# jie0530/act-plus-plus

Hardware: AMD Instinct MI355X
Metric: policy steps/sec (4x480x640 cams, chunk=100, bs=8) (higher is better)
Workload: dtype f32 (f16x3 split products: 3 fp16 MFMAs per fp32 product, fp32 accumulate); 1 GPU; ACT eval policy query: 4 cams 480x640 u8, chunk 100, hidden 512, ff 3200, 4 enc + 7 dec layers (layer 0 live), per-GPU batch 8, + temporal ensemble; per_gpu_batch=8, global_batch=8, parallelism=replicas x1

## Files before the change

act-plus-plus_amd/csrc/attn.hip:

```cpp
#include "common.h"
#include "dropout.h"
#include "split16.h"
#include <cstdio>
#include <cstdlib>

namespace {

constexpr bool ATTN_NOPF = true;
constexpr int KT = 64;
typedef _Float16 h16x8 __attribute__((ext_vector_type(8)));

__device__ __forceinline__ void attn_block_coords(int& bx, int& by, int& bz) {
    const int gx = gridDim.x, gy = gridDim.y;
    const int total = gx * gy * (int)gridDim.z;
    const int lin = ((int)blockIdx.z * gy + (int)blockIdx.y) * gx + (int)blockIdx.x;
    const int xcd = lin & 7, q = total >> 3, r = total & 7;
    const int base = (xcd < r) ? xcd * (q + 1) : r * (q + 1) + (xcd - r) * q;
    const int flat = base + (lin >> 3);
    bx = flat % gx;
    const int rest = flat / gx;
    by = rest % gy;
    bz = rest / gy;
}

template <int HD>
__global__ __launch_bounds__(256) void attn_f32_kernel(AttnArgs p, int nsplit, int chunk) {
    constexpr int HH = HD / 2;
    constexpr int DT = (HD + 31) / 32;
    constexpr int VD = DT * 32;
    constexpr int KS = HD + 4;
    __shared__ __attribute__((aligned(16))) float s_k[KT * KS];
    __shared__ __attribute__((aligned(16))) float s_v[KT * VD];

    const int t = threadIdx.x, lane = t & 63, wave = t >> 6;
    const int li = lane & 31, lh = lane >> 5;
    int bx, h, b;
    attn_block_coords(bx, h, b);
    const int split = bx % nsplit;
    const int q = (bx / nsplit) * 128 + wave * 32 + li;
    const int k_begin = split * chunk;
    const int k_end = (k_begin + chunk < p.Nk) ? k_begin + chunk : p.Nk;
    const bool qok = q < p.Nq;

    const float qscale = p.scale * 1.4426950408889634f;
    const float* Qp = p.Q + (int64_t)b * p.q_bs + (int64_t)(qok ? q : 0) * p.q_rs + h * HD + lh * HH;
    float qreg[HH];
#pragma unroll
    for (int s = 0; s < HH; s += 4) {
        f32x4 v = *reinterpret_cast<const f32x4*>(Qp + s);
#pragma unroll
        for (int j = 0; j < 4; ++j) qreg[s + j] = qok ? v[j] * qscale : 0.f;
    }
    const float* Kb = p.K + (int64_t)b * p.k_bs + h * HD;
    const float* Vb = p.V + (int64_t)b * p.v_bs + h * HD;
    const uint8_t* kpm = p.kpm ? p.kpm + (int64_t)b * p.kpm_bs : nullptr;

    f32x16 O[DT];
#pragma unroll
    for (int d = 0; d < DT; ++d)
#pragma unroll
        for (int e = 0; e < 16; ++e) O[d][e] = 0.f;
    float m_run = -INFINITY, l_run = 0.f;

    if (HD < VD) {
        for (int e = t; e < KT * VD; e += 256) s_v[e] = 0.f;
        __syncthreads();
    }

    __shared__ uint8_t s_dead[KT];
    constexpr int C4 = HD / 4;
    constexpr int NLD = (KT * C4 + 255) / 256;
    f32x4 pk[NLD], pv[NLD];
    auto fetch = [&](int kt0) {
#pragma unroll
        for (int i = 0; i < NLD; ++i) {
            const int e = t + 256 * i;
            const int kr = e / C4, c = e - kr * C4;
            const int key = kt0 + kr;
            const bool ok = e < KT * C4 && key < k_end;
            const int64_t koff = ok ? (int64_t)key * p.k_rs + c * 4 : 0;
            const int64_t voff = ok ? (int64_t)key * p.v_rs + c * 4 : 0;
            const f32x4 kv = *reinterpret_cast<const f32x4*>(Kb + koff);
            const f32x4 vv = *reinterpret_cast<const f32x4*>(Vb + voff);
            const f32x4 z = {0.f, 0.f, 0.f, 0.f};
            pk[i] = ok ? kv : z;
            pv[i] = ok ? vv : z;
        }
    };
    fetch(k_begin);
    for (int kt0 = k_begin; kt0 < k_end; kt0 += KT) {
#pragma unroll
        for (int i = 0; i < NLD; ++i) {
            const int e = t + 256 * i;
            if (e < KT * C4) {
                const int kr = e / C4, c = e - kr * C4;
                *reinterpret_cast<f32x4*>(&s_k[kr * KS + c * 4]) = pk[i];
                *reinterpret_cast<f32x4*>(&s_v[kr * VD + c * 4]) = pv[i];
            }
        }
        const bool ragged = kt0 + KT > k_end || kpm != nullptr;
        if (ragged && t < KT) {
            const int key = kt0 + t;
            s_dead[t] = (key >= k_end) || (kpm && kpm[key] != 0);
        }
        __syncthreads();
        if (kt0 + KT < k_end) fetch(kt0 + KT);
#pragma unroll
        for (int sub = 0; sub < KT / 32; ++sub) {
            const int kb = kt0 + sub * 32;
            if (kb < k_end) {
                f32x16 S;
#pragma unroll
                for (int e = 0; e < 16; ++e) S[e] = 0.f;
                const float* krow = &s_k[(sub * 32 + li) * KS + lh * HH];
#pragma unroll
                for (int s = 0; s < HH; s += 4) {
                    const f32x4 kv = *reinterpret_cast<const f32x4*>(krow + s);
#pragma unroll
                    for (int j = 0; j < 4; ++j)
                        S = __builtin_amdgcn_mfma_f32_32x32x2f32(kv[j], qreg[s + j], S, 0, 0, 0);
                }
                if (ragged) {
#pragma unroll
                    for (int e = 0; e < 16; ++e)
                        if (s_dead[sub * 32 + (e & 3) + 8 * (e >> 2) + 4 * lh]) S[e] = -INFINITY;
                }
                if (p.causal) {
#pragma unroll
                    for (int e = 0; e < 16; ++e)
                        if (kb + (e & 3) + 8 * (e >> 2) + 4 * lh > q) S[e] = -INFINITY;
                }
                float mt = S[0];
#pragma unroll
                for (int e = 1; e < 16; ++e) mt = fmaxf(mt, S[e]);
                mt = fmaxf(mt, __shfl_xor(mt, 32, 64));
                const float m_new = fmaxf(m_run, mt);
                const float m_safe = (m_new == -INFINITY) ? 0.f : m_new;
                const float alpha = __builtin_amdgcn_exp2f(m_run - m_safe);
                float rs = 0.f;
#pragma unroll
                for (int e = 0; e < 16; ++e) {
                    S[e] = __builtin_amdgcn_exp2f(S[e] - m_safe);
                    rs += S[e];
                }
                rs += __shfl_xor(rs, 32, 64);
                l_run = l_run * alpha + rs;
                m_run = m_new;
                if (p.drop_p > 0.f) {
                    const float ds = 1.f / (1.f - p.drop_p);
                    const uint64_t rowbase = (((uint64_t)b * p.H + h) * p.Nq + (qok ? q : 0)) * (uint64_t)p.Nk;
#pragma unroll
                    for (int e = 0; e < 16; ++e) {
                        const int key = kb + (e & 3) + 8 * (e >> 2) + 4 * lh;
                        S[e] = actmi_keep(p.drop_seed, rowbase + key, p.drop_p) ? S[e] * ds : 0.f;
                    }
                }
#pragma unroll
                for (int d = 0; d < DT; ++d)
#pragma unroll
                    for (int e = 0; e < 16; ++e) O[d][e] *= alpha;
#pragma unroll
                for (int e = 0; e < 16; ++e) {
                    const int kl = sub * 32 + (e & 3) + 8 * (e >> 2) + 4 * lh;
#pragma unroll
                    for (int d = 0; d < DT; ++d) {
                        const float vv = s_v[kl * VD + d * 32 + li];
                        O[d] = __builtin_amdgcn_mfma_f32_32x32x2f32(vv, S[e], O[d], 0, 0, 0);
                    }
                }
            }
        }
        __syncthreads();
    }
    if (qok) {
        if (nsplit == 1) {
            const float inv = 1.f / l_run;
            float* Op = p.O + (int64_t)b * p.o_bs + (int64_t)q * p.o_rs + h * HD;
#pragma unroll
            for (int d = 0; d < DT; ++d)
#pragma unroll
                for (int g = 0; g < 4; ++g) {
                    const int d0 = d * 32 + 8 * g + 4 * lh;
                    if (d0 < HD) {
                        f32x4 o = {O[d][4 * g] * inv, O[d][4 * g + 1] * inv, O[d][4 * g + 2] * inv, O[d][4 * g + 3] * inv};
                        *reinterpret_cast<f32x4*>(Op + d0) = o;
                    }
                }
            if (p.lse && lh == 0) p.lse[((int64_t)b * p.H + h) * p.Nq + q] = m_run * 0.6931471805599453f + logf(l_run);
        } else {
            const int64_t row = (((int64_t)split * p.B + b) * p.H + h) * p.Nq + q;
            float* Op = p.ws + row * HD;
            float* ml = p.ws + (int64_t)nsplit * p.B * p.H * p.Nq * HD + row * 2;
#pragma unroll
            for (int d = 0; d < DT; ++d)
#pragma unroll
                for (int g = 0; g < 4; ++g) {
                    const int d0 = d * 32 + 8 * g + 4 * lh;
                    if (d0 < HD) {
                        f32x4 o = {O[d][4 * g], O[d][4 * g + 1], O[d][4 * g + 2], O[d][4 * g + 3]};
                        *reinterpret_cast<f32x4*>(Op + d0) = o;
                    }
                }
            if (lh == 0) { ml[0] = m_run; ml[1] = l_run; }
        }
    }
}

template <int HD>
__global__ __launch_bounds__(256, 3) void attn_f16x3_kernel(AttnArgs p, int nsplit, int chunk) {
    constexpr int NS = HD / 16;
    constexpr int DT = (HD + 31) / 32;
    constexpr int VD = DT * 32;
    constexpr int KROW = 4 * HD + 16;
    constexpr int VROW = 4 * KT + 16;
    __shared__ __attribute__((aligned(16))) unsigned char s_k[KT * KROW];
    __shared__ __attribute__((aligned(16))) unsigned char s_vt[VD * VROW];
    __shared__ uint8_t s_dead[KT];

    const int t = threadIdx.x, lane = t & 63, wave = t >> 6;
    const int li = lane & 31, lh = lane >> 5;
    int bx, h, b;
    attn_block_coords(bx, h, b);
    const int split = bx % nsplit;
    const int q = (bx / nsplit) * 128 + wave * 32 + li;
    const int k_begin = split * chunk;
    const int k_end = (k_begin + chunk < p.Nk) ? k_begin + chunk : p.Nk;
    const bool qok = q < p.Nq;

    const float qscale = p.scale * 1.4426950408889634f;
    const float* Qp = p.Q + (int64_t)b * p.q_bs + (int64_t)(qok ? q : 0) * p.q_rs + h * HD + lh * 8;
    h16x8 qh[NS], ql[NS];
#pragma unroll
    for (int s = 0; s < NS; ++s) {
        f32x4 v0 = *reinterpret_cast<const f32x4*>(Qp + s * 16);
        f32x4 v1 = *reinterpret_cast<const f32x4*>(Qp + s * 16 + 4);
        const float sc = qok ? qscale : 0.f;
        v0 *= sc; v1 *= sc;
        uint2 h0, l0, h1, l1;
        split16(v0, h0, l0);
        split16(v1, h1, l1);
        qh[s] = __builtin_bit_cast(h16x8, uint4{h0.x, h0.y, h1.x, h1.y});
        ql[s] = __builtin_bit_cast(h16x8, uint4{l0.x, l0.y, l1.x, l1.y});
    }
    const float* Kb = p.K + (int64_t)b * p.k_bs + h * HD;
    const float* Vb = p.V + (int64_t)b * p.v_bs + h * HD;
    const uint8_t* kpm = p.kpm ? p.kpm + (int64_t)b * p.kpm_bs : nullptr;

    f32x16 O[DT];
#pragma unroll
    for (int d = 0; d < DT; ++d)
#pragma unroll
        for (int e = 0; e < 16; ++e) O[d][e] = 0.f;
    float m_run = -INFINITY, l_run = 0.f;

    if (HD < VD) {
        for (int e = t; e < VD * VROW / 4; e += 256) reinterpret_cast<uint32_t*>(s_vt)[e] = 0u;
        __syncthreads();
    }

    constexpr int C4 = HD / 4;
    constexpr int NLK = (KT * C4 + 255) / 256;
    constexpr int NLV = (KT / 2 * C4 + 255) / 256;
    f32x4 pk[NLK], pv[NLV][2];
    auto vc = [&](int e) { return ((e >> 5) % (C4 / 4)) * 4 + (e & 3); };
    auto vkp = [&](int e) { return ((e >> 5) / (C4 / 4)) * 8 + ((e >> 2) & 7); };
    auto fetch = [&](int kt0) {
        const f32x4 z = {0.f, 0.f, 0.f, 0.f};
#pragma unroll
        for (int i = 0; i < NLK; ++i) {
            const int e = t + 256 * i;
            const int kr = e / C4, c = e - kr * C4;
            const int key = kt0 + kr;
            const bool ok = e < KT * C4 && key < k_end;
            const f32x4 kv = *reinterpret_cast<const f32x4*>(Kb + (ok ? (int64_t)key * p.k_rs + c * 4 : 0));
            pk[i] = ok ? kv : z;
        }
#pragma unroll
        for (int i = 0; i < NLV; ++i) {
            const int e = t + 256 * i;
            const int kp = vkp(e), c = vc(e);
#pragma unroll
            for (int u = 0; u < 2; ++u) {
                const int key = kt0 + 2 * kp + u;
                const bool ok = e < KT / 2 * C4 && key < k_end;
                const f32x4 vv = *reinterpret_cast<const f32x4*>(Vb + (ok ? (int64_t)key * p.v_rs + c * 4 : 0));
                pv[i][u] = ok ? vv : z;
            }
        }
    };
    if (!ATTN_NOPF) fetch(k_begin);
    for (int kt0 = k_begin; kt0 < k_end; kt0 += KT) {
        if (ATTN_NOPF) fetch(kt0);
#pragma unroll
        for (int i = 0; i < NLK; ++i) {
            const int e = t + 256 * i;
            if (e < KT * C4) {
                const int kr = e / C4, c = e - kr * C4;
                uint2 hi, lo;
                split16(pk[i], hi, lo);
                *reinterpret_cast<uint2*>(s_k + kr * KROW + c * 8) = hi;
                *reinterpret_cast<uint2*>(s_k + kr * KROW + 2 * HD + c * 8) = lo;
            }
        }
#pragma unroll
        for (int i = 0; i < NLV; ++i) {
            const int e = t + 256 * i;
            if (e < KT / 2 * C4) {
                const int kp = vkp(e), c = vc(e);
                uint2 ha, la, hb, lb;
                split16(pv[i][0], ha, la);
                split16(pv[i][1], hb, lb);
                const int kl = 2 * kp, r = kl & 15;
                const int pos = (kl & ~15) | (r & 3) | ((r & 8) >> 1) | ((r & 4) << 1);
                unsigned char* dst = s_vt + (c * 4) * VROW + pos * 2;
                *reinterpret_cast<uint32_t*>(dst + 0 * VROW) = (ha.x & 0xffffu) | (hb.x << 16);
                *reinterpret_cast<uint32_t*>(dst + 1 * VROW) = (ha.x >> 16) | (hb.x & 0xffff0000u);
                *reinterpret_cast<uint32_t*>(dst + 2 * VROW) = (ha.y & 0xffffu) | (hb.y << 16);
                *reinterpret_cast<uint32_t*>(dst + 3 * VROW) = (ha.y >> 16) | (hb.y & 0xffff0000u);
                *reinterpret_cast<uint32_t*>(dst + 0 * VROW + 2 * KT) = (la.x & 0xffffu) | (lb.x << 16);
                *reinterpret_cast<uint32_t*>(dst + 1 * VROW + 2 * KT) = (la.x >> 16) | (lb.x & 0xffff0000u);
                *reinterpret_cast<uint32_t*>(dst + 2 * VROW + 2 * KT) = (la.y & 0xffffu) | (lb.y << 16);
                *reinterpret_cast<uint32_t*>(dst + 3 * VROW + 2 * KT) = (la.y >> 16) | (lb.y & 0xffff0000u);
            }
        }
        const bool ragged = kt0 + KT > k_end || kpm != nullptr;
        if (ragged && t < KT) {
            const int key = kt0 + t;
            s_dead[t] = (key >= k_end) || (kpm && kpm[key] != 0);
        }
        __syncthreads();
        if (!ATTN_NOPF && kt0 + KT < k_end) fetch(kt0 + KT);
#pragma unroll
        for (int sub = 0; sub < KT / 32; ++sub) {
            const int kb = kt0 + sub * 32;
            if (kb < k_end) {
                f32x16 S;
#pragma unroll
                for (int e = 0; e < 16; ++e) S[e] = 0.f;
                const unsigned char* krow = s_k + (sub * 32 + li) * KROW + lh * 16;
#pragma unroll
                for (int s = 0; s < NS; ++s) {
                    const h16x8 kh = __builtin_bit_cast(h16x8, *reinterpret_cast<const f32x4*>(krow + s * 32));
                    const h16x8 kl = __builtin_bit_cast(h16x8, *reinterpret_cast<const f32x4*>(krow + 2 * HD + s * 32));
                    S = __builtin_amdgcn_mfma_f32_32x32x16_f16(kl, qh[s], S, 0, 0, 0);
                    S = __builtin_amdgcn_mfma_f32_32x32x16_f16(kh, ql[s], S, 0, 0, 0);
                    S = __builtin_amdgcn_mfma_f32_32x32x16_f16(kh, qh[s], S, 0, 0, 0);
                }
                if (ragged) {
#pragma unroll
                    for (int e = 0; e < 16; ++e)
                        if (s_dead[sub * 32 + (e & 3) + 8 * (e >> 2) + 4 * lh]) S[e] = -INFINITY;
                }
                if (p.causal) {
#pragma unroll
                    for (int e = 0; e < 16; ++e)
                        if (kb + (e & 3) + 8 * (e >> 2) + 4 * lh > q) S[e] = -INFINITY;
                }
                float mt = S[0];
#pragma unroll
                for (int e = 1; e < 16; ++e) mt = fmaxf(mt, S[e]);
                mt = fmaxf(mt, __shfl_xor(mt, 32, 64));
                const float m_new = fmaxf(m_run, mt);
                const float m_safe = (m_new == -INFINITY) ? 0.f : m_new;
                const float alpha = __builtin_amdgcn_exp2f(m_run - m_safe);
                float rs = 0.f;
#pragma unroll
                for (int e = 0; e < 16; ++e) {
                    S[e] = __builtin_amdgcn_exp2f(S[e] - m_safe);
                    rs += S[e];
                }
                rs += __shfl_xor(rs, 32, 64);
                l_run = l_run * alpha + rs;
                m_run = m_new;
                if (p.drop_p > 0.f) {
                    const float ds = 1.f / (1.f - p.drop_p);
                    const uint64_t rowbase = (((uint64_t)b * p.H + h) * p.Nq + (qok ? q : 0)) * (uint64_t)p.Nk;
#pragma unroll
                    for (int e = 0; e < 16; ++e) {
                        const int key = kb + (e & 3) + 8 * (e >> 2) + 4 * lh;
                        S[e] = actmi_keep(p.drop_seed, rowbase + key, p.drop_p) ? S[e] * ds : 0.f;
                    }
                }
                h16x8 ph[2], pl[2];
#pragma unroll
                for (int g2 = 0; g2 < 2; ++g2) {
                    const f32x4 a0 = {S[8 * g2], S[8 * g2 + 1], S[8 * g2 + 2], S[8 * g2 + 3]};
                    const f32x4 a1 = {S[8 * g2 + 4], S[8 * g2 + 5], S[8 * g2 + 6], S[8 * g2 + 7]};
                    uint2 h0, l0, h1, l1;
                    split16(a0, h0, l0);
                    split16(a1, h1, l1);
                    ph[g2] = __builtin_bit_cast(h16x8, uint4{h0.x, h0.y, h1.x, h1.y});
                    pl[g2] = __builtin_bit_cast(h16x8, uint4{l0.x, l0.y, l1.x, l1.y});
                }
#pragma unroll
                for (int d = 0; d < DT; ++d) {
#pragma unroll
                    for (int e = 0; e < 16; ++e) O[d][e] *= alpha;
                    const unsigned char* vrow = s_vt + (d * 32 + li) * VROW + sub * 64 + lh * 16;
#pragma unroll
                    for (int g2 = 0; g2 < 2; ++g2) {
                        const h16x8 vh = __builtin_bit_cast(h16x8, *reinterpret_cast<const f32x4*>(vrow + g2 * 32));
                        const h16x8 vl = __builtin_bit_cast(h16x8, *reinterpret_cast<const f32x4*>(vrow + 2 * KT + g2 * 32));
                        O[d] = __builtin_amdgcn_mfma_f32_32x32x16_f16(vl, ph[g2], O[d], 0, 0, 0);
                        O[d] = __builtin_amdgcn_mfma_f32_32x32x16_f16(vh, pl[g2], O[d], 0, 0, 0);
                        O[d] = __builtin_amdgcn_mfma_f32_32x32x16_f16(vh, ph[g2], O[d], 0, 0, 0);
                    }
                }
            }
        }
        __syncthreads();
    }
    if (qok) {
        if (nsplit == 1) {
            const float inv = 1.f / l_run;
            float* Op = p.O + (int64_t)b * p.o_bs + (int64_t)q * p.o_rs + h * HD;
#pragma unroll
            for (int d = 0; d < DT; ++d)
#pragma unroll
                for (int g = 0; g < 4; ++g) {
                    const int d0 = d * 32 + 8 * g + 4 * lh;
                    if (d0 < HD) {
                        f32x4 o = {O[d][4 * g] * inv, O[d][4 * g + 1] * inv, O[d][4 * g + 2] * inv, O[d][4 * g + 3] * inv};
                        *reinterpret_cast<f32x4*>(Op + d0) = o;
                    }
                }
            if (p.lse && lh == 0) p.lse[((int64_t)b * p.H + h) * p.Nq + q] = m_run * 0.6931471805599453f + logf(l_run);
        } else {
            const int64_t row = (((int64_t)split * p.B + b) * p.H + h) * p.Nq + q;
            float* Op = p.ws + row * HD;
            float* ml = p.ws + (int64_t)nsplit * p.B * p.H * p.Nq * HD + row * 2;
#pragma unroll
            for (int d = 0; d < DT; ++d)
#pragma unroll
                for (int g = 0; g < 4; ++g) {
                    const int d0 = d * 32 + 8 * g + 4 * lh;
                    if (d0 < HD) {
                        f32x4 o = {O[d][4 * g], O[d][4 * g + 1], O[d][4 * g + 2], O[d][4 * g + 3]};
                        *reinterpret_cast<f32x4*>(Op + d0) = o;
                    }
                }
            if (lh == 0) { ml[0] = m_run; ml[1] = l_run; }
        }
    }
}


__global__ void attn_combine_kernel(AttnArgs p, int nsplit, int HD) {
    const int64_t idx = (int64_t)blockIdx.x * blockDim.x + threadIdx.x;
    const int D4 = HD / 4;
    const int64_t total = (int64_t)p.B * p.H * p.Nq * D4;
    if (idx >= total) return;
    const int d4 = (int)(idx % D4);
    const int64_t bhq = idx / D4;
    const int q = (int)(bhq % p.Nq);
    const int h = (int)((bhq / p.Nq) % p.H);
    const int b = (int)(bhq / ((int64_t)p.Nq * p.H));
    const int64_t per = (int64_t)p.B * p.H * p.Nq;
    const float* mlb = p.ws + (int64_t)nsplit * per * HD;
    float m = -INFINITY;
    for (int s = 0; s < nsplit; ++s) m = fmaxf(m, mlb[(s * per + bhq) * 2]);
    const float msafe = (m == -INFINITY) ? 0.f : m;
    float L = 0.f;
    f32x4 acc = {0.f, 0.f, 0.f, 0.f};
    for (int s = 0; s < nsplit; ++s) {
        const float w = __builtin_amdgcn_exp2f(mlb[(s * per + bhq) * 2] - msafe);
        L += mlb[(s * per + bhq) * 2 + 1] * w;
        acc += *reinterpret_cast<const f32x4*>(p.ws + (s * per + bhq) * HD + d4 * 4) * w;
    }
    const float inv = 1.f / L;
    *reinterpret_cast<f32x4*>(p.O + (int64_t)b * p.o_bs + (int64_t)q * p.o_rs + h * HD + d4 * 4) = acc * inv;
    if (p.lse && d4 == 0) p.lse[bhq] = msafe * 0.6931471805599453f + logf(L);
}

}

int launch_attention(const AttnArgs& a, hipStream_t st, std::string* err) {
    auto fail = [&](const char* m) { if (err) *err = std::string("attention: ") + m; return -2; };
    if (a.B <= 0 || a.Nq <= 0) return 0;
    if (a.Nk <= 0) return fail("Nk must be positive");
    if (a.causal && a.Nq != a.Nk) return fail("causal needs Nq == Nk");
    if ((a.q_rs & 3) || (a.k_rs & 3) || (a.v_rs & 3) || (a.o_rs & 3) || (a.q_bs & 3) || (a.k_bs & 3) || (a.v_bs & 3) ||
        (a.o_bs & 3))
        return fail("strides must be multiples of 4 floats");
    if (((uintptr_t)a.Q & 15) || ((uintptr_t)a.K & 15) || ((uintptr_t)a.V & 15) || ((uintptr_t)a.O & 15))
        return fail("pointers must be 16-byte aligned");
    static const int env_prec = env_gemm_prec(ACTMI_PREC_F32);
    const int prec = a.prec ? a.prec : env_prec;
    if (prec != ACTMI_PREC_F32 && prec != ACTMI_PREC_F16X3) return fail("bad prec");
    const bool f16 = prec == ACTMI_PREC_F16X3;
    const int qblocks = (a.Nq + 127) / 128;
    const int tiles = (a.Nk + KT - 1) / KT;
    int nsplit = 1;
    if (a.ws) {
        const long blocks = (long)qblocks * a.H * a.B;
        static const long target = getenv("ACTMI_ATTN_SPLIT_TARGET") ? atol(getenv("ACTMI_ATTN_SPLIT_TARGET")) : 1024;
        nsplit = (int)((target + blocks - 1) / blocks);
        if (nsplit < 1) nsplit = 1;
        if (nsplit > 8) nsplit = 8;
        if (nsplit > tiles / 2) nsplit = tiles / 2 > 0 ? tiles / 2 : 1;
        while (nsplit > 1 && (int64_t)nsplit * a.B * a.Nq * ((int64_t)a.H * a.HD + 2 * a.H) > a.ws_floats) --nsplit;
    }
    const int chunk = ((tiles + nsplit - 1) / nsplit) * KT;
    dim3 grid(qblocks * nsplit, a.H, a.B);
    if (prof_enabled()) {
        char nm[48];
        snprintf(nm, sizeof(nm), "attn_%s_kernel<%d>", f16 ? "f16x3" : "f32", a.HD);
        prof_begin(nm, 4.0 * a.B * a.H * (double)a.Nq * a.Nk * a.HD,
                   4.0 * a.B * a.H * a.HD * (2.0 * a.Nq + 2.0 * a.Nk), st);
    }
    if (f16) {
        switch (a.HD) {
            case 64: hipLaunchKernelGGL(attn_f16x3_kernel<64>, grid, dim3(256), 0, st, a, nsplit, chunk); break;
            case 32: hipLaunchKernelGGL(attn_f16x3_kernel<32>, grid, dim3(256), 0, st, a, nsplit, chunk); break;
            case 16: hipLaunchKernelGGL(attn_f16x3_kernel<16>, grid, dim3(256), 0, st, a, nsplit, chunk); break;
            default: return fail("head_dim must be 16, 32 or 64");
        }
    } else
    switch (a.HD) {
        case 64: hipLaunchKernelGGL(attn_f32_kernel<64>, grid, dim3(256), 0, st, a, nsplit, chunk); break;
        case 32: hipLaunchKernelGGL(attn_f32_kernel<32>, grid, dim3(256), 0, st, a, nsplit, chunk); break;
        case 16: hipLaunchKernelGGL(attn_f32_kernel<16>, grid, dim3(256), 0, st, a, nsplit, chunk); break;
        default: return fail("head_dim must be 16, 32 or 64");
    }
    if (nsplit > 1) {
        const int64_t total = (int64_t)a.B * a.H * a.Nq * (a.HD / 4);
        hipLaunchKernelGGL(attn_combine_kernel, dim3((unsigned)((total + 255) / 256)), dim3(256), 0, st, a, nsplit, a.HD);
    }
    prof_end(st);
    hipError_t e = hipGetLastError();
    if (e != hipSuccess) { if (err) *err = std::string("attention launch: ") + hipGetErrorString(e); return -3; }
    return 0;
}
```

Baseline: 1812 policy steps/s.

## Specialize attention key tiles into interior fast path with packed math and MFMA priority

Splits the key-tile loop into an interior variant for full tiles with no mask, causal or dropout, which skips bounds checks, the dead-key mask and dropout logic and uses precomputed 32-bit offsets for the K/V loads. It also adds a paired fp16 split using v_fma_mix for the V transpose, packed f32x2 scaling and exp, and s_setprio around the MFMA blocks. The aim is to cut VALU and address overhead around the matrix ops. The cost is extra code size and two instantiations of the tile body, which can raise register pressure.

```diff
diff --git a/act-plus-plus_amd/csrc/attn.hip b/act-plus-plus_amd/csrc/attn.hip
--- a/act-plus-plus_amd/csrc/attn.hip
+++ b/act-plus-plus_amd/csrc/attn.hip
@@ -3,12 +3,37 @@
 #include "split16.h"
 #include <cstdio>
 #include <cstdlib>
+#include <type_traits>
 
 namespace {
 
-constexpr bool ATTN_NOPF = true;
 constexpr int KT = 64;
 typedef _Float16 h16x8 __attribute__((ext_vector_type(8)));
+
+__device__ __forceinline__ void split16_pair(const f32x4 a, const f32x4 b, uint32_t (&hi)[4], uint32_t (&lo)[4]) {
+#pragma unroll
+    for (int j = 0; j < 4; ++j) {
+        const f32x2 ab = {a[j], b[j]};
+        const unsigned h = __builtin_bit_cast(unsigned, __builtin_convertvector(ab, h16x2));
+        float r0, r1;
+        asm("v_fma_mix_f32 %0, %1, -1.0, %2 op_sel:[0,0,0] op_sel_hi:[1,0,0]" : "=v"(r0) : "v"(h), "v"(a[j]));
+        asm("v_fma_mix_f32 %0, %1, -1.0, %2 op_sel:[1,0,0] op_sel_hi:[1,0,0]" : "=v"(r1) : "v"(h), "v"(b[j]));
+        const f32x2 r = {r0, r1};
+        hi[j] = h;
+        lo[j] = __builtin_bit_cast(unsigned, __builtin_convertvector(r, h16x2));
+    }
+}
+
+__device__ __forceinline__ void scale16(f32x16& o, const float a) {
+    const f32x2 a2 = {a, a};
+#pragma unroll
+    for (int e = 0; e < 16; e += 2) {
+        f32x2 x = {o[e], o[e + 1]};
+        x *= a2;
+        o[e] = x[0];
+        o[e + 1] = x[1];
+    }
+}
 
 __device__ __forceinline__ void attn_block_coords(int& bx, int& by, int& bz) {
     const int gx = gridDim.x, gy = gridDim.y;
@@ -259,85 +284,101 @@
     }
 
     constexpr int C4 = HD / 4;
-    constexpr int NLK = (KT * C4 + 255) / 256;
+    constexpr int NLK = KT * C4 / 256;
     constexpr int NLV = (KT / 2 * C4 + 255) / 256;
-    f32x4 pk[NLK], pv[NLV][2];
+    constexpr bool VALL = KT / 2 * C4 >= 256;
+    static_assert(KT * C4 % 256 == 0 && 256 % C4 == 0 && (NLV == 1 || C4 == 16), "item -> (key, chunk) decomposition below");
     auto vc = [&](int e) { return ((e >> 5) % (C4 / 4)) * 4 + (e & 3); };
     auto vkp = [&](int e) { return ((e >> 5) / (C4 / 4)) * 8 + ((e >> 2) & 7); };
-    auto fetch = [&](int kt0) {
-        const f32x4 z = {0.f, 0.f, 0.f, 0.f};
+    constexpr int KSTEP = 256 / C4;
+    constexpr int VSTEP = 2 * 8 * 8 / (C4 / 4);
+    const int k_kr = t / C4, k_c = t % C4;
+    const int v_kl = 2 * vkp(t), v_c = vc(t), v_r = v_kl & 15;
+    const int v_pos = (v_kl & ~15) | (v_r & 3) | ((v_r & 8) >> 1) | ((v_r & 4) << 1);
+    unsigned char* const k_dst = s_k + k_kr * KROW + k_c * 8;
+    unsigned char* const v_dst = s_vt + (v_c * 4) * VROW + v_pos * 2;
+    const bool v_item = VALL || t < KT / 2 * C4;
+    const uint32_t k_goff = ((uint32_t)k_kr * (uint32_t)p.k_rs + k_c * 4) * 4u;
+    const uint32_t v_goff = ((uint32_t)v_kl * (uint32_t)p.v_rs + v_c * 4) * 4u;
+    const int64_t k_tile = (int64_t)KT * p.k_rs, v_tile = (int64_t)KT * p.v_rs;
+    const float* Kt = Kb + (int64_t)k_begin * p.k_rs;
+    const float* Vt = Vb + (int64_t)k_begin * p.v_rs;
+    const bool plain = kpm == nullptr && !p.causal && !(p.drop_p > 0.f) && (uint32_t)p.k_rs < (1u << 24) &&
+                       (uint32_t)p.v_rs < (1u << 24);
+
+    auto tile = [&](const int kt0, auto interiorc) {
+        constexpr bool INTERIOR = decltype(interiorc)::value;
+        f32x4 pk[NLK], pv[NLV][2];
+        if constexpr (INTERIOR) {
+            uint32_t kg = k_goff, vg = v_goff;
+            asm volatile("" : "+v"(kg), "+v"(vg));
+#pragma unroll
+            for (int i = 0; i < NLK; ++i)
+                pk[i] = *reinterpret_cast<const f32x4*>(reinterpret_cast<const char*>(Kt + (int64_t)(i * KSTEP) * p.k_rs) + kg);
+            if (v_item) {
+#pragma unroll
+                for (int i = 0; i < NLV; ++i)
+#pragma unroll
+                    for (int u = 0; u < 2; ++u)
+                        pv[i][u] = *reinterpret_cast<const f32x4*>(
+                            reinterpret_cast<const char*>(Vt + (int64_t)(i * VSTEP + u) * p.v_rs) + vg);
+            }
+        } else {
+            const f32x4 z = {0.f, 0.f, 0.f, 0.f};
+#pragma unroll
+            for (int i = 0; i < NLK; ++i) {
+                const int key = kt0 + k_kr + i * KSTEP;
+                const bool ok = key < k_end;
+                const f32x4 kv = *reinterpret_cast<const f32x4*>(Kb + (ok ? (int64_t)key * p.k_rs + k_c * 4 : 0));
+                pk[i] = ok ? kv : z;
+            }
+#pragma unroll
+            for (int i = 0; i < NLV; ++i)
+#pragma unroll
+                for (int u = 0; u < 2; ++u) {
+                    const int key = kt0 + v_kl + i * VSTEP + u;
+                    const bool ok = v_item && key < k_end;
+                    const f32x4 vv = *reinterpret_cast<const f32x4*>(Vb + (ok ? (int64_t)key * p.v_rs + v_c * 4 : 0));
+                    pv[i][u] = ok ? vv : z;
+                }
+        }
 #pragma unroll
         for (int i = 0; i < NLK; ++i) {
-            const int e = t + 256 * i;
-            const int kr = e / C4, c = e - kr * C4;
-            const int key = kt0 + kr;
-            const bool ok = e < KT * C4 && key < k_end;
-            const f32x4 kv = *reinterpret_cast<const f32x4*>(Kb + (ok ? (int64_t)key * p.k_rs + c * 4 : 0));
-            pk[i] = ok ? kv : z;
-        }
-#pragma unroll
-        for (int i = 0; i < NLV; ++i) {
-            const int e = t + 256 * i;
-            const int kp = vkp(e), c = vc(e);
-#pragma unroll
-            for (int u = 0; u < 2; ++u) {
-                const int key = kt0 + 2 * kp + u;
-                const bool ok = e < KT / 2 * C4 && key < k_end;
-                const f32x4 vv = *reinterpret_cast<const f32x4*>(Vb + (ok ? (int64_t)key * p.v_rs + c * 4 : 0));
-                pv[i][u] = ok ? vv : z;
-            }
-        }
-    };
-    if (!ATTN_NOPF) fetch(k_begin);
-    for (int kt0 = k_begin; kt0 < k_end; kt0 += KT) {
-        if (ATTN_NOPF) fetch(kt0);
-#pragma unroll
-        for (int i = 0; i < NLK; ++i) {
-            const int e = t + 256 * i;
-            if (e < KT * C4) {
-                const int kr = e / C4, c = e - kr * C4;
-                uint2 hi, lo;
-                split16(pk[i], hi, lo);
-                *reinterpret_cast<uint2*>(s_k + kr * KROW + c * 8) = hi;
-                *reinterpret_cast<uint2*>(s_k + kr * KROW + 2 * HD + c * 8) = lo;
-            }
-        }
-#pragma unroll
-        for (int i = 0; i < NLV; ++i) {
-            const int e = t + 256 * i;
-            if (e < KT / 2 * C4) {
-                const int kp = vkp(e), c = vc(e);
-                uint2 ha, la, hb, lb;
-                split16(pv[i][0], ha, la);
-                split16(pv[i][1], hb, lb);
-                const int kl = 2 * kp, r = kl & 15;
-                const int pos = (kl & ~15) | (r & 3) | ((r & 8) >> 1) | ((r & 4) << 1);
-                unsigned char* dst = s_vt + (c * 4) * VROW + pos * 2;
-                *reinterpret_cast<uint32_t*>(dst + 0 * VROW) = (ha.x & 0xffffu) | (hb.x << 16);
-                *reinterpret_cast<uint32_t*>(dst + 1 * VROW) = (ha.x >> 16) | (hb.x & 0xffff0000u);
-                *reinterpret_cast<uint32_t*>(dst + 2 * VROW) = (ha.y & 0xffffu) | (hb.y << 16);
-                *reinterpret_cast<uint32_t*>(dst + 3 * VROW) = (ha.y >> 16) | (hb.y & 0xffff0000u);
-                *reinterpret_cast<uint32_t*>(dst + 0 * VROW + 2 * KT) = (la.x & 0xffffu) | (lb.x << 16);
-                *reinterpret_cast<uint32_t*>(dst + 1 * VROW + 2 * KT) = (la.x >> 16) | (lb.x & 0xffff0000u);
-                *reinterpret_cast<uint32_t*>(dst + 2 * VROW + 2 * KT) = (la.y & 0xffffu) | (lb.y << 16);
-                *reinterpret_cast<uint32_t*>(dst + 3 * VROW + 2 * KT) = (la.y >> 16) | (lb.y & 0xffff0000u);
-            }
-        }
-        const bool ragged = kt0 + KT > k_end || kpm != nullptr;
-        if (ragged && t < KT) {
-            const int key = kt0 + t;
-            s_dead[t] = (key >= k_end) || (kpm && kpm[key] != 0);
+            uint2 hi, lo;
+            split16(pk[i], hi, lo);
+            *reinterpret_cast<uint2*>(k_dst + i * KSTEP * KROW) = hi;
+            *reinterpret_cast<uint2*>(k_dst + i * KSTEP * KROW + 2 * HD) = lo;
+        }
+        if (v_item) {
+#pragma unroll
+            for (int i = 0; i < NLV; ++i) {
+                uint32_t hi[4], lo[4];
+                split16_pair(pv[i][0], pv[i][1], hi, lo);
+                unsigned char* dst = v_dst + i * VSTEP * 2;
+#pragma unroll
+                for (int j = 0; j < 4; ++j) {
+                    *reinterpret_cast<uint32_t*>(dst + j * VROW) = hi[j];
+                    *reinterpret_cast<uint32_t*>(dst + j * VROW + 2 * KT) = lo[j];
+                }
+            }
+        }
+        const bool ragged = !INTERIOR && (kt0 + KT > k_end || kpm != nullptr);
+        if constexpr (!INTERIOR) {
+            if (ragged && t < KT) {
+                const int key = kt0 + t;
+                s_dead[t] = (key >= k_end) || (kpm && kpm[key] != 0);
+            }
         }
         __syncthreads();
-        if (!ATTN_NOPF && kt0 + KT < k_end) fetch(kt0 + KT);
 #pragma unroll
         for (int sub = 0; sub < KT / 32; ++sub) {
             const int kb = kt0 + sub * 32;
-            if (kb < k_end) {
+            if (INTERIOR || kb < k_end) {
                 f32x16 S;
 #pragma unroll
                 for (int e = 0; e < 16; ++e) S[e] = 0.f;
                 const unsigned char* krow = s_k + (sub * 32 + li) * KROW + lh * 16;
+                __builtin_amdgcn_s_setprio(1);
 #pragma unroll
                 for (int s = 0; s < NS; ++s) {
                     const h16x8 kh = __builtin_bit_cast(h16x8, *reinterpret_cast<const f32x4*>(krow + s * 32));
@@ -346,15 +387,18 @@
                     S = __builtin_amdgcn_mfma_f32_32x32x16_f16(kh, ql[s], S, 0, 0, 0);
                     S = __builtin_amdgcn_mfma_f32_32x32x16_f16(kh, qh[s], S, 0, 0, 0);
                 }
-                if (ragged) {
-#pragma unroll
-                    for (int e = 0; e < 16; ++e)
-                        if (s_dead[sub * 32 + (e & 3) + 8 * (e >> 2) + 4 * lh]) S[e] = -INFINITY;
-                }
-                if (p.causal) {
-#pragma unroll
-                    for (int e = 0; e < 16; ++e)
-                        if (kb + (e & 3) + 8 * (e >> 2) + 4 * lh > q) S[e] = -INFINITY;
+                __builtin_amdgcn_s_setprio(0);
+                if constexpr (!INTERIOR) {
+                    if (ragged) {
+#pragma unroll
+                        for (int e = 0; e < 16; ++e)
+                            if (s_dead[sub * 32 + (e & 3) + 8 * (e >> 2) + 4 * lh]) S[e] = -INFINITY;
+                    }
+                    if (p.causal) {
+#pragma unroll
+                        for (int e = 0; e < 16; ++e)
+                            if (kb + (e & 3) + 8 * (e >> 2) + 4 * lh > q) S[e] = -INFINITY;
+                    }
                 }
                 float mt = S[0];
 #pragma unroll
@@ -363,22 +407,29 @@
                 const float m_new = fmaxf(m_run, mt);
                 const float m_safe = (m_new == -INFINITY) ? 0.f : m_new;
                 const float alpha = __builtin_amdgcn_exp2f(m_run - m_safe);
-                float rs = 0.f;
-#pragma unroll
-                for (int e = 0; e < 16; ++e) {
-                    S[e] = __builtin_amdgcn_exp2f(S[e] - m_safe);
-                    rs += S[e];
-                }
+                const f32x2 m2 = {m_safe, m_safe};
+                f32x2 rs2 = {0.f, 0.f};
+#pragma unroll
+                for (int e = 0; e < 16; e += 2) {
+                    const f32x2 x = f32x2{S[e], S[e + 1]} - m2;
+                    const f32x2 y = {__builtin_amdgcn_exp2f(x[0]), __builtin_amdgcn_exp2f(x[1])};
+                    S[e] = y[0];
+                    S[e + 1] = y[1];
+                    rs2 = e ? rs2 + y : y;
+                }
+                float rs = rs2[0] + rs2[1];
                 rs += __shfl_xor(rs, 32, 64);
                 l_run = l_run * alpha + rs;
                 m_run = m_new;
-                if (p.drop_p > 0.f) {
-                    const float ds = 1.f / (1.f - p.drop_p);
-                    const uint64_t rowbase = (((uint64_t)b * p.H + h) * p.Nq + (qok ? q : 0)) * (uint64_t)p.Nk;
-#pragma unroll
-                    for (int e = 0; e < 16; ++e) {
-                        const int key = kb + (e & 3) + 8 * (e >> 2) + 4 * lh;
-                        S[e] = actmi_keep(p.drop_seed, rowbase + key, p.drop_p) ? S[e] * ds : 0.f;
+                if constexpr (!INTERIOR) {
+                    if (p.drop_p > 0.f) {
+                        const float ds = 1.f / (1.f - p.drop_p);
+                        const uint64_t rowbase = (((uint64_t)b * p.H + h) * p.Nq + (qok ? q : 0)) * (uint64_t)p.Nk;
+#pragma unroll
+                        for (int e = 0; e < 16; ++e) {
+                            const int key = kb + (e & 3) + 8 * (e >> 2) + 4 * lh;
+                            S[e] = actmi_keep(p.drop_seed, rowbase + key, p.drop_p) ? S[e] * ds : 0.f;
+                        }
                     }
                 }
                 h16x8 ph[2], pl[2];
@@ -392,10 +443,10 @@
                     ph[g2] = __builtin_bit_cast(h16x8, uint4{h0.x, h0.y, h1.x, h1.y});
                     pl[g2] = __builtin_bit_cast(h16x8, uint4{l0.x, l0.y, l1.x, l1.y});
                 }
+                __builtin_amdgcn_s_setprio(1);
 #pragma unroll
                 for (int d = 0; d < DT; ++d) {
-#pragma unroll
-                    for (int e = 0; e < 16; ++e) O[d][e] *= alpha;
+                    scale16(O[d], alpha);
                     const unsigned char* vrow = s_vt + (d * 32 + li) * VROW + sub * 64 + lh * 16;
 #pragma unroll
                     for (int g2 = 0; g2 < 2; ++g2) {
@@ -406,9 +457,16 @@
                         O[d] = __builtin_amdgcn_mfma_f32_32x32x16_f16(vh, ph[g2], O[d], 0, 0, 0);
                     }
                 }
+                __builtin_amdgcn_s_setprio(0);
             }
         }
         __syncthreads();
+    };
+    for (int kt0 = k_begin; kt0 < k_end; kt0 += KT) {
+        if (plain && kt0 + KT <= k_end) tile(kt0, std::true_type{});
+        else tile(kt0, std::false_type{});
+        Kt += k_tile;
+        Vt += v_tile;
     }
     if (qok) {
         if (nsplit == 1) {
```

New measurement: 1821 policy steps/s, median of 6. No clear change (+0.5%).
